# magcks/opencl_raytracer

Hardware: AMD Instinct MI355X
Metric: Mrays/s at 1920×1080 (bunny.off, sibenik.off); PGM bit-exact vs CPU (higher is better)
Workload: dtype f32; 1 GPU; bunny.off 1920x1080 -s 1 -a 3 (primary + 28 AO rays per hit sub-pixel), longest-axis BVH; rays_per_frame=34404360, primary_hits=1154670, parallelism=image bands x1, frames_in_flight=1, frame_launch=hipGraph replay, pgm_md5=e02eaeb53640206897ce798cda5cbd83, pgm_matches_golden=True, scene_bytes_on_device=20837632, scene_copies_on_device=1, triangles=70570, device=AMD Radeon Graphics

## Files before the change

include/rt_hip_debug.h:

```cpp
#ifndef RT_HIP_DEBUG_H
#define RT_HIP_DEBUG_H

#include "rt_hip_ring.h"

#ifdef __cplusplus
extern "C" {
#endif

double rt_total_kernel_ms(const rt_host *h);
float rt_last_ao_ms(const rt_host *h);
double rt_total_ao_ms(const rt_host *h);
uint64_t rt_kernel_launches(const rt_host *h);
void rt_reset_timers(rt_host *h);

int rt_ring_device_bytes(const rt_ring *r, uint64_t *scene_bytes, uint32_t *scene_copies, uint64_t *total_bytes);

int rt_ring_calibration(const rt_ring *r, float *ms_without, float *ms_with, int *prefetch_in_use);
int rt_set_ao_prefetch(rt_host *h, int on);

int rt_walk_entries(rt_host *h, uint32_t *tiles_hit, uint32_t *tiles_narrowed, double *mean_share, double *mean_packet_share);

int rt_ring_reset_clock(rt_ring *r);
int rt_ring_keep_frame_times(rt_ring *r, int on);
int rt_ring_frame_times(const rt_ring *r, uint64_t frame, float ms[4]);

int rt_ring_timers(rt_ring *r, double *kernel_ms, uint64_t *frames, double *ao_ms, uint64_t *ao_frames);
void rt_ring_reset_timers(rt_ring *r);

int rt_ring_cpu_times(const rt_ring *r, double *submit_s, double *wait_s, double *collect_s, uint64_t *frames);

int rt_ring_rccl_info(rt_ring *r, int *comm_ranks, int *rccl_version);
int rt_ring_rccl_self_test(rt_ring *r);

int rt_debug_measure_tile_costs(rt_host *h, uint32_t frames, int reorder);
int rt_debug_set_order_policy(rt_host *h, float heavy, float runway, float split_above);
int rt_debug_set_primary_split(rt_host *h, uint32_t above);
uint32_t rt_debug_tile_order_slots(rt_host *h);
uint32_t rt_debug_tiles(rt_host *h);
int rt_debug_tile_order(rt_host *h, uint32_t *order, uint32_t *constants24, uint32_t *tile_words, float *tile_costs);
int rt_debug_set_tile_order(rt_host *h, const uint32_t *order, uint32_t slots, const uint32_t *constants24);
int rt_debug_split_tiles(rt_host *h, uint32_t out[8]);
int rt_debug_set_cheap_claims(rt_host *h, float cheap_below);
int rt_debug_cheap_tiles(rt_host *h, uint32_t out[8]);

int rt_debug_prune_facts(rt_host *h, float *prune_margin, uint32_t *unpruned_bytes, uint32_t *primary_bytes);

int rt_debug_poison_hit_list(rt_host *h);

int rt_debug_set_views_chunk(rt_host *h, uint32_t max_views);
int rt_debug_last_views(rt_host *h, uint32_t *views, uint32_t *chunks, uint64_t *ao_points);

#define RT_DEBUG_NEAREST_NO_START 1u
#define RT_DEBUG_NEAREST_NO_PRUNE 2u
// ... 19 lines not shown
```

opencl_raytracer_amd/api.py:

```python
from __future__ import annotations

import ctypes as C
import weakref
import os
import sys
from typing import Optional

import numpy as np

_HERE = os.path.dirname(os.path.abspath(__file__))


def lib_path() -> str:
    return os.path.join(_HERE, os.environ.get("OCRT_LIB_DIR", "lib"), "libocrt_hip.so")


class RtError(RuntimeError):
    def __init__(self, code: int, message: str):
        super().__init__(f"[rt {code}] {message}")
        self.code = code
        self.message = message


RT_E_INVALID, RT_E_NO_DEVICE, RT_E_DEVICE, RT_E_STATE, RT_E_IO = -1, -2, -3, -4, -5
# ... 149 lines not shown
    "rt_ring_submit": (C.c_int, [C.c_void_p, C.POINTER(C.c_uint64)]),
    "rt_ring_collect": (C.c_int, [C.c_void_p, C.POINTER(C.c_uint64), C.POINTER(C.c_uint32), C.POINTER(C.c_void_p)]),
    "rt_ring_collect_into_device": (C.c_int, [C.c_void_p, C.c_void_p]),
    "rt_ring_step": (C.c_int, [C.c_void_p]),
    "rt_ring_run": (C.c_int, [C.c_void_p, C.c_uint32]),
    "rt_ring_drain": (C.c_int, [C.c_void_p]),
    "rt_ring_last_image_device": (C.c_int, [C.c_void_p, C.POINTER(C.c_void_p)]),
    "rt_ring_download_last": (C.c_int, [C.c_void_p, C.c_void_p]),
    "rt_ring_reset_clock": (C.c_int, [C.c_void_p]),
    "rt_ring_keep_frame_times": (C.c_int, [C.c_void_p, C.c_int]),
    "rt_ring_frame_times": (C.c_int, [C.c_void_p, C.c_uint64, C.POINTER(C.c_float)]),
    "rt_ring_timers": (C.c_int, [C.c_void_p, C.POINTER(C.c_double), C.POINTER(C.c_uint64), C.POINTER(C.c_double),
                                 C.POINTER(C.c_uint64)]),
    "rt_ring_reset_timers": (None, [C.c_void_p]),
    "rt_ring_cpu_times": (C.c_int, [C.c_void_p, C.POINTER(C.c_double), C.POINTER(C.c_double), C.POINTER(C.c_double),
                                    C.POINTER(C.c_uint64)]),
    "rt_rccl_available": (C.c_int, []),
    "rt_rccl_unique_id": (C.c_int, [C.c_void_p]),
    "rt_ring_attach_rccl": (C.c_int, [C.c_void_p, C.c_void_p]),
    "rt_ring_rccl_self_test": (C.c_int, [C.c_void_p]),
    "rt_print_info": (None, []),
    "rt_device_count": (C.c_int, []),
    "rt_debug_measure_tile_costs": (C.c_int, [C.c_void_p, C.c_uint32, C.c_int]),
    "rt_debug_set_order_policy": (C.c_int, [C.c_void_p, C.c_float, C.c_float, C.c_float]),
    "rt_debug_set_primary_split": (C.c_int, [C.c_void_p, C.c_uint32]),
    "rt_debug_tile_order_slots": (C.c_uint32, [C.c_void_p]),
    "rt_debug_tiles": (C.c_uint32, [C.c_void_p]),
    "rt_debug_tile_order": (C.c_int, [C.c_void_p, C.c_void_p, C.c_void_p, C.c_void_p, C.c_void_p]),
    "rt_debug_set_tile_order": (C.c_int, [C.c_void_p, C.c_void_p, C.c_uint32, C.c_void_p]),
    "rt_debug_split_tiles": (C.c_int, [C.c_void_p, C.c_void_p]),
    "rt_debug_set_cheap_claims": (C.c_int, [C.c_void_p, C.c_float]),
    "rt_debug_cheap_tiles": (C.c_int, [C.c_void_p, C.c_void_p]),
    "rt_debug_prune_facts": (C.c_int, [C.c_void_p, C.c_void_p, C.c_void_p, C.c_void_p]),
    "rt_debug_poison_hit_list": (C.c_int, [C.c_void_p]),
    "rt_debug_node_test_forms": (C.c_int, [C.c_int, C.c_void_p, C.c_uint32, C.c_void_p, C.c_uint32, C.c_void_p]),
    "rt_debug_set_views_chunk": (C.c_int, [C.c_void_p, C.c_uint32]),
    "rt_debug_last_views": (C.c_int, [C.c_void_p, C.POINTER(C.c_uint32), C.POINTER(C.c_uint32), C.POINTER(C.c_uint64)]),
    "rt_trace_closest": (C.c_int, [C.c_void_p, C.c_void_p, C.c_void_p, C.c_uint32, C.c_float, C.c_uint32, C.c_void_p]),
    "rt_trace_occluded": (C.c_int, [C.c_void_p, C.c_void_p, C.c_void_p, C.c_uint32, C.c_float, C.c_uint32, C.c_void_p]),
    "rt_trace_closest_device": (C.c_int, [C.c_void_p, C.c_void_p, C.c_void_p, C.c_uint32, C.c_float, C.c_uint32, C.c_void_p,
                                          C.c_void_p]),
    "rt_trace_occluded_device": (C.c_int, [C.c_void_p, C.c_void_p, C.c_void_p, C.c_uint32, C.c_float, C.c_uint32, C.c_void_p,
                                           C.c_void_p]),
    "rt_last_query_ms": (C.c_float, [C.c_void_p]),
    "rt_segments_occluded": (C.c_int, [C.c_void_p, C.c_void_p, C.c_void_p, C.c_uint32, C.c_float, C.c_float, C.c_uint32, C.c_void_p]),
    "rt_segments_closest": (C.c_int, [C.c_void_p, C.c_void_p, C.c_void_p, C.c_uint32, C.c_float, C.c_float, C.c_uint32, C.c_void_p]),
    "rt_segments_occluded_device": (C.c_int, [C.c_void_p, C.c_void_p, C.c_void_p, C.c_uint32, C.c_float, C.c_float, C.c_uint32,
                                              C.c_void_p, C.c_void_p]),
    "rt_segments_closest_device": (C.c_int, [C.c_void_p, C.c_void_p, C.c_void_p, C.c_uint32, C.c_float, C.c_float, C.c_uint32,
                                             C.c_void_p, C.c_void_p]),
    "rt_visibility_masks": (C.c_int, [C.c_void_p, C.c_void_p, C.c_uint32, C.c_void_p, C.c_uint32, C.c_float, C.c_float, C.c_uint32,
                                      C.c_void_p]),
    "rt_visibility_masks_device": (C.c_int, [C.c_void_p, C.c_void_p, C.c_uint32, C.c_void_p, C.c_uint32, C.c_float, C.c_float,
                                             C.c_uint32, C.c_void_p, C.c_void_p]),
    "rt_instances_segments_occluded": (C.c_int, [C.c_void_p, C.c_void_p, C.c_void_p, C.c_uint32, C.c_float, C.c_float, C.c_uint32,
                                                 C.c_void_p]),
    "rt_instances_segments_closest": (C.c_int, [C.c_void_p, C.c_void_p, C.c_void_p, C.c_uint32, C.c_float, C.c_float, C.c_uint32,
                                                C.c_void_p]),
    "rt_instances_segments_occluded_device": (C.c_int, [C.c_void_p, C.c_void_p, C.c_void_p, C.c_uint32, C.c_float, C.c_float, C.c_uint32,
                                                        C.c_void_p, C.c_void_p]),
    "rt_instances_segments_closest_device": (C.c_int, [C.c_void_p, C.c_void_p, C.c_void_p, C.c_uint32, C.c_float, C.c_float, C.c_uint32,
                                                       C.c_void_p, C.c_void_p]),
    "rt_instances_visibility_masks": (C.c_int, [C.c_void_p, C.c_void_p, C.c_uint32, C.c_void_p, C.c_uint32, C.c_float, C.c_float,
                                                C.c_uint32, C.c_void_p]),
    "rt_instances_visibility_masks_device": (C.c_int, [C.c_void_p, C.c_void_p, C.c_uint32, C.c_void_p, C.c_uint32, C.c_float, C.c_float,
                                                       C.c_uint32, C.c_void_p, C.c_void_p]),
# ... 591 lines not shown
        words, costs = np.zeros(tiles, np.uint32), np.zeros(tiles, np.float32)
        _check(lib.rt_debug_tile_order(self._h, order.ctypes.data, constants.ctypes.data, words.ctypes.data, costs.ctypes.data))
        return {"order": order, "constants": constants.reshape(8, 3), "words": words, "costs": costs}

    def set_tile_order(self, order, constants) -> None:
        order = np.ascontiguousarray(order, np.uint32)
        constants = np.ascontiguousarray(constants, np.uint32).reshape(24)
        _check(load_library().rt_debug_set_tile_order(self._h, order.ctypes.data, len(order), constants.ctypes.data))

    def split_tiles(self) -> np.ndarray:
        out = np.zeros(8, np.uint32)
        _check(load_library().rt_debug_split_tiles(self._h, out.ctypes.data))
        return out

    def set_cheap_claims(self, cheap_below: float) -> None:
        _check(load_library().rt_debug_set_cheap_claims(self._h, float(cheap_below)))

    def cheap_tiles(self) -> np.ndarray:
        out = np.zeros(8, np.uint32)
        _check(load_library().rt_debug_cheap_tiles(self._h, out.ctypes.data))
        return out

    def prune_facts(self) -> dict:
        margin, unpruned, primary = C.c_float(), C.c_uint32(), C.c_uint32()
        _check(load_library().rt_debug_prune_facts(self._h, C.byref(margin), C.byref(unpruned), C.byref(primary)))
        return {"prune_margin": float(margin.value), "unpruned_bytes": unpruned.value, "primary_bytes": primary.value}

    def walk_entries(self) -> dict:
        hit, narrowed, share, packet_share = C.c_uint32(), C.c_uint32(), C.c_double(), C.c_double()
        _check(load_library().rt_walk_entries(self._h, C.byref(hit), C.byref(narrowed), C.byref(share), C.byref(packet_share)))
        return {"tiles_hit": hit.value, "tiles_narrowed": narrowed.value, "mean_share": share.value,
                "mean_packet_share": packet_share.value}

    def stats(self) -> dict:
        s = _Stats()
        _check(load_library().rt_get_stats(self._h, C.byref(s)))
        return {k: int(getattr(s, k)) for k, _ in _Stats._fields_}

    @property
    def last_kernel_ms(self) -> float:
        return float(load_library().rt_last_kernel_ms(self._h))

    @property
    def total_kernel_ms(self) -> float:
        return float(load_library().rt_total_kernel_ms(self._h))

    @property
    def last_ao_ms(self) -> float:
        return float(load_library().rt_last_ao_ms(self._h))

    @property
    def total_ao_ms(self) -> float:
        return float(load_library().rt_total_ao_ms(self._h))

    @property
    def kernel_launches(self) -> int:
        return int(load_library().rt_kernel_launches(self._h))

    def reset_timers(self) -> None:
        load_library().rt_reset_timers(self._h)

    def trace_closest(self, origins, directions, max_distance: float = 100000.0, outputs=QUERY_OUTPUTS, sort: bool = True) -> dict:
        return self._trace(True, origins, directions, max_distance, tuple(outputs), sort)

    def trace_occluded(self, origins, directions, max_distance: float = 100000.0, sort: bool = True):
        return self._trace(False, origins, directions, max_distance, ("hit",), sort)["hit"]
# ... 668 lines not shown
```

opencl_raytracer_amd/csrc/c_api.cc:

```cpp
#include "../../include/rt_hip.h"
#include "../../include/rt_hip_ao.h"
#include "../../include/rt_hip_camera.h"
#include "../../include/rt_hip_directional.h"
#include "../../include/rt_hip_layers.h"
#include "../../include/rt_hip_debug.h"
#include "../../include/rt_hip_multihit.h"
#include "../../include/rt_hip_nearest.h"
#include "../../include/rt_hip_query.h"
#include "../../include/rt_hip_segment.h"
#include "../../include/rt_hip_instance_build.h"
#include "../../include/rt_hip_instance_directional.h"
#include "../../include/rt_hip_instance_multihit.h"
#include "../../include/rt_hip_instance_nearest.h"
#include "../../include/rt_hip_instance_segments.h"
#include "../../include/rt_hip_instance_views.h"
#include "../../include/rt_hip_instances.h"
#include "../../include/rt_hip_views.h"
#include "../../include/rt_hip_update.h"
#include "../../include/rt_hip_build.h"

#include <algorithm>
#include <hip/hip_runtime.h>

#include <cmath>
// ... 545 lines not shown

int rt_ring_set_calibration(rt_ring *r, int on) {
	if (!r)
		return fail(RT_E_INVALID, "null argument");
	r->ring->setCalibration(on != 0);
	return RT_OK;
}

int rt_ring_calibration(const rt_ring *r, float *ms_without, float *ms_with, int *prefetch_in_use) {
	if (!r)
		return fail(RT_E_INVALID, "null argument");
	if (ms_without)
		*ms_without = r->ring->calibrationMs()[0];
	if (ms_with)
		*ms_with = r->ring->calibrationMs()[1];
	if (prefetch_in_use)
		*prefetch_in_use = r->ring->aoPrefetch() ? 1 : 0;
	return RT_OK;
}

int rt_walk_entries(rt_host *h, uint32_t *tiles_hit, uint32_t *tiles_narrowed, double *mean_share, double *mean_packet_share) {
	if (!h)
		return fail(RT_E_INVALID, "null argument");
	return guarded([&] {
		const ocrt::DeviceRenderer::WalkEntries e = h->dev->walkEntries();
		if (tiles_hit)
			*tiles_hit = e.tiles_hit;
		if (tiles_narrowed)
			*tiles_narrowed = e.tiles_narrowed;
		if (mean_share)
			*mean_share = e.mean_share;
		if (mean_packet_share)
			*mean_packet_share = e.mean_packet_share;
	});
}

int rt_set_ao_prefetch(rt_host *h, int on) {
	if (!h)
		return fail(RT_E_INVALID, "null argument");
	return guarded([&] { h->dev->setAoPrefetch(on != 0); });
}

int rt_debug_measure_tile_costs(rt_host *h, uint32_t frames, int reorder) {
	if (!h)
		return fail(RT_E_INVALID, "null argument");
	return guarded([&] {
		h->dev->measureTileCosts(frames, reorder != 0);
	});
}

int rt_debug_set_primary_split(rt_host *h, uint32_t above) {
	if (!h)
		return fail(RT_E_INVALID, "null argument");
	return guarded([&] { h->dev->setPrimarySplit(above); });
}

int rt_debug_set_order_policy(rt_host *h, float heavy, float runway, float split_above) {
	if (!h)
		return fail(RT_E_INVALID, "null argument");
	return guarded([&] { h->dev->setOrderPolicy(heavy, runway, split_above); });
}

uint32_t rt_debug_tile_order_slots(rt_host *h) {
	if (!h)
		return 0;
	std::vector<uint32_t> order, constants, words;
// ... 1285 lines not shown
```

opencl_raytracer_amd/csrc/device_renderer.cc:

```cpp
#include "device_internal.h"

#include <algorithm>
#include <array>
#include <atomic>
#include <chrono>

#include <hip/hip_runtime.h>

#include <cstddef>
#include <cstdio>
#include <cstdlib>
#include <cstring>
#include <mutex>
#include <sstream>

namespace ocrt {


int visible_device_count() {
	int count = 0;
	if (hipGetDeviceCount(&count) != hipSuccess)
		return 0;
	return count;
}
// ... 430 lines not shown
	OCRT_HIP(hipStreamSynchronize((hipStream_t) stream));
	const double whole = (double) kp.node_count * sizeof(NodeRec);
	double sum = 0.0, sum_packets = 0.0;
	unsigned long long packets = 0;
	const size_t tiles_per_piece = std::max<size_t>(1, ((size_t) 32 << 20) / (stride * 2 * sizeof(uint32_t)));
	std::vector<uint32_t> ranges;
	for (size_t first = 0; first < tile_count; first += tiles_per_piece) {
		const size_t count = std::min(tiles_per_piece, tile_count - first);
		ranges.resize(count * stride * 2);
		OCRT_HIP(hipMemcpyAsync(ranges.data(), (const uint32_t *) d_tile_entry + first * stride * 2, ranges.size() * sizeof(uint32_t), hipMemcpyDeviceToHost,
		                        (hipStream_t) stream));
		OCRT_HIP(hipStreamSynchronize((hipStream_t) stream));
		for (size_t t = first; t < first + count; ++t) {
			if ((words[t] & 0xFFu) == 0u)
				continue;
			++out.tiles_hit;
			const uint32_t *const of_tile = &ranges[2 * stride * (t - first)];
			const double bytes = std::min(whole, (double) of_tile[1]) - (double) of_tile[0];
			out.tiles_narrowed += of_tile[0] != 0u || bytes < whole;
			sum += bytes / whole;
			const bool per_direction = (words[t] & 0xFFu) == 64u && kp.ao_mode == AO_UNIFORM && stride > 1;
			for (size_t k = 1; k <= kp.ao_dirs; ++k) {
				const uint32_t *const r = per_direction ? of_tile + 2 * k : of_tile;
				sum_packets += (std::min(whole, (double) r[1]) - (double) r[0]) / whole;
				++packets;
			}
		}
	}
	out.mean_share = out.tiles_hit ? sum / out.tiles_hit : 1.0;
	out.mean_packet_share = packets ? sum_packets / (double) packets : 1.0;
	return out;
}

void DeviceRenderer::expectFrames(uint64_t frames) {
	const bool before = expected_frames >= FRAMES_WORTH_INTERVALS, after = frames >= FRAMES_WORTH_INTERVALS;
	if (before != after && scene_ready)
		requireFramePath("expectFrames");
	expected_frames = frames;
	if (before == after || !scene_ready)
		return;
	std::shared_ptr<const DeviceScene> scene = scene_on_device;
	std::shared_ptr<DeviceScene> mine = scene_of_my_own;
	adopt(std::move(scene));
	scene_of_my_own = std::move(mine);
}

void DeviceRenderer::setAoPrefetch(bool on) {
	if (on == ao_prefetch)
		return;
	ao_prefetch = on;
	++scene_version;
}

bool DeviceRenderer::calibrateAoPrefetch(float *ms_without, float *ms_with) {
	if (!scene_ready)
		throw std::logic_error("calibration before upload");
	requireFramePath("calibration");
	const bool has_ao = kp.ao_mode == AO_UNIFORM && kp.ao_dirs > 0 && tile_count > 0 && kp.fast_walk && kp.walk_scale > 0.0f;
	float median[2] = { 0.0f, 0.0f };
	if (has_ao) {
		const bool before = ao_prefetch;
		std::vector<float> samples[2];
		for (int round = 0; round < 6; ++round)
			for (int form = 0; form < 2; ++form) {
				ao_prefetch = form != 0;
				enqueueRender();
// ... 321 lines not shown
```

opencl_raytracer_amd/csrc/device_renderer.h:

```cpp
#pragma once
#include <array>
#include <cstdint>
#include <memory>
#include <stdexcept>
#include <string>
#include <vector>

#include "device_types.h"
#include "ray_tracer.h"
#include "scene_pack.h"

namespace ocrt {

struct DeviceError : std::runtime_error {
	using std::runtime_error::runtime_error;
};

int visible_device_count();
void warm_up_device(int device);

class DeviceScene {
	public:
		static std::shared_ptr<DeviceScene> create(int device, const PackedScene &scene, const RayTracer::Options &options, bool for_a_stream = true,
		                                           const float *eye = nullptr);
// ... 75 lines not shown
		void setRefitGroup(uint32_t nodes) { refit_group = nodes; }
		uint32_t refitGroup() const { return refit_group; }
		void setCamera(const CameraPose &pose);
		bool cameraIsSet() const { return pose_set; }
		const CameraPose &camera() const { return pose; }

		void enqueueRender();
		void enqueueResize();
		void enqueueResizeInto(void *device_u8);
		void enqueueFrame(void *device_u8 = nullptr);
		void prepareFrame(void *device_u8 = nullptr);
		void setGraphMode(bool on) { graph_mode = on; }
		bool sceneReady() const { return scene_ready; }
		bool graphMode() const { return graph_mode; }
		void synchronize();
		void waitForStream();
		void setEpochEvent(void *event) { epoch_event = event; }
		void setKeepStamps(bool on) { keep_stamps = on; }
		const float *lastFrameTimes() const { return last_times; }

		const void *deviceBands() const { return d_u8; }
		void *streamHandle() const { return stream; }
		void setDeviceShare(unsigned hosts) {
			device_share = hosts < 1u ? 1u : hosts;
			kp.shared_device = device_share > 1u ? 1 : 0;
		}
		void setAoPrefetch(bool on);
		struct WalkEntries {
			uint32_t tiles_hit, tiles_narrowed;
			double mean_share;
			double mean_packet_share;
		};
		WalkEntries walkEntries() const;
		bool aoPrefetch() const { return ao_prefetch; }
		static constexpr uint64_t FRAMES_WORTH_INTERVALS = 16;
		static constexpr float CHEAP_BELOW_DEFAULT = 0.15f;
		void expectFrames(uint64_t frames);
		uint64_t expectedFrames() const { return expected_frames; }
		bool walkIntervalsInUse() const { return intervals_in_use; }
		bool measureTileCosts(unsigned frames = 2, bool reorder = true);
		void takeOrderFrom(const DeviceRenderer &other);
		bool orderIsMeasured() const { return tile_cost.size() == tile_count && tile_count != 0; }
		void setOrderPolicy(float heavy, float runway, float split_above = -1.0f);
		void setPrimarySplit(uint32_t above);
		void poisonHitList();
		void tileOrder(std::vector<uint32_t> &order, std::vector<uint32_t> &constants, std::vector<uint32_t> &words, std::vector<float> &cost) const;
		void setTileOrder(const std::vector<uint32_t> &order, const std::vector<uint32_t> &constants);
		const std::array<uint32_t, XCD_GROUPS> &splitTiles() const { return split_tiles; }
		const std::array<uint32_t, XCD_GROUPS> &cheapTiles() const { return cheap_tiles; }
		void setCheapClaims(float cheap_below);
		bool calibrateAoPrefetch(float *ms_without = nullptr, float *ms_with = nullptr);
		uint32_t aoWorkgroups() const {
			if (scene_beyond_caches)
				return compute_units * 8u;
			return device_share >= 6u ? compute_units * 3u : device_share > 1u ? compute_units * 9u / 2u : compute_units * 8u;
		}
		uint32_t globalRowOf(uint32_t local_row) const;

		void downloadFloat(float *host_image);
		void downloadResizedLocal(unsigned char *host);
		void downloadResizedFull(unsigned char *host);

		void setStream(void *hip_stream);
		void usePrivateStream();

		RenderStats stats();
// ... 136 lines not shown
```

opencl_raytracer_amd/csrc/kernels/entry.hip.h:

```cpp
#pragma once
#include "common.hip.h"

namespace ocrt {

constexpr uint32_t ENTRY_WAVES = 4;
__global__ __launch_bounds__(64 * ENTRY_WAVES) void entry_kernel(const NodeRec *__restrict__ walk, const HitRec *__restrict__ hits,
                                                                 const uint32_t *__restrict__ tile_hits, const uint32_t *__restrict__ tile_base,
                                                                 const float4 *__restrict__ ao_table, uint2 *__restrict__ tile_entry,
                                                                 uint32_t tiles, uint32_t stride, int32_t uniform_table,
                                                                 float max_distance) {
	__shared__ float origin[ENTRY_WAVES][3][64];
	__shared__ float frame[ENTRY_WAVES][9][64];
	const uint32_t wave = threadIdx.x >> 6, lane = threadIdx.x & 63u;
	const uint32_t tile = blockIdx.x * ENTRY_WAVES + wave;
	if (tile >= tiles)
		return;
	const uint32_t hit_count = tile_hits[tile] & 0xFFu;
	uint2 *const out = tile_entry + (size_t) tile * stride;
	const uint32_t whole = walk[0].skip / (uint32_t) sizeof(NodeRec);
	if (lane < hit_count) {
		const HitRec rec = hits[(size_t) tile_base[tile] + lane];
		const float nx = rec.nx, ny = rec.ny, nz = rec.nz;
		const float eps = 1.0f / 100000.0f;
		origin[wave][0][lane] = rec.ox + nx * eps;
// ... 38 lines not shown
			return !(box.lo[0] - box.hi[0] > hi[0] || box.lo[0] + box.hi[0] < lo[0] || box.lo[1] - box.hi[1] > hi[1] || box.lo[1] + box.hi[1] < lo[1] ||
			         box.lo[2] - box.hi[2] > hi[2] || box.lo[2] + box.hi[2] < lo[2]);
		};
		uint32_t begin = 0u, end = whole ? whole : 1u;
		if (!odd && (j == 0u || one_direction)) {
			uint32_t n = 0u;
			while (skip_of(n) > 1u) {
				uint32_t first = 0u, index = 0u, others = 0u;
				for (uint32_t c = n + 1u; c < n + skip_of(n); c += skip_of(c)) {
					if (first)
						others += meets(c) ? 1u : 0u;
					else {
						++index;
						if (meets(c))
							first = c;
					}
				}
				if (first == 0u) {
					n += skip_of(n);
					break;
				}
				if (index == 1u && others != 0u)
					break;
				n = first;
			}
			begin = n;
			n = 0u;
			while (skip_of(n) > 1u) {
				uint32_t last = 0u;
				for (uint32_t c = n + 1u; c < n + skip_of(n); c += skip_of(c))
					if (meets(c))
						last = c;
				if (last == 0u) {
					end = n;
					break;
				}
				end = last + skip_of(last);
				n = last;
			}
			if (begin > end)
				begin = end;
		}
		out[j] = make_uint2(begin * (uint32_t) sizeof(NodeRec), end * (uint32_t) sizeof(NodeRec));
	}
}

}
```

opencl_raytracer_amd/csrc/kernels/walk.hip.h:

```cpp
#pragma once
#include "common.hip.h"

namespace ocrt {

__device__ __forceinline__ bool exact_box(const float4 lo, const float4 hi, const Ray &ray, float max_distance, bool alive,
                                          uint32_t at, uint32_t skip, uint32_t &mine) {
	const bool here = alive && mine == at;
	const bool box = here && slab_hit(lo, hi, ray, max_distance);
	mine = here ? (box ? at + 1u : at + skip) : mine;
	return box;
}

struct SignMasks {
	unsigned long long x, y, z;
};
__device__ __forceinline__ SignMasks sign_masks(const Ray &r) {
	SignMasks m;
	m.x = wave_ballot(r.ix >= 0.0f);
	m.y = wave_ballot(r.iy >= 0.0f);
	m.z = wave_ballot(r.iz >= 0.0f);
	return m;
}

typedef unsigned int u32x8 __attribute__((ext_vector_type(8)));
// ... 33 lines not shown
	"\tv_max_f32 v58, 1, v58\n"                    \
	"\tv_min_f32 v61, %[below], v61\n"             \
	"\tv_max3_f32 v56, v56, v57, v58\n"            \
	"\tv_min3_f32 v59, v59, v60, v61\n"            \
	"\tv_cmp_le_f32 vcc, v56, v59\n"
#define OCRT_TEST_MIXED(LX, LY, LZ, HX, HY, HZ)    \
	"\tv_fma_f32 v56, " LX ", %[ix], %[oix]\n"     \
	"\tv_fma_f32 v57, " HX ", %[ix], %[oix]\n"     \
	"\tv_fma_f32 v58, " LY ", %[iy], %[oiy]\n"     \
	"\tv_fma_f32 v59, " HY ", %[iy], %[oiy]\n"     \
	"\tv_fma_f32 v60, " LZ ", %[iz], %[oiz]\n"     \
	"\tv_fma_f32 v61, " HZ ", %[iz], %[oiz]\n"     \
	"\tv_cndmask_b32 v62, v57, v56, %[px]\n"       \
	"\tv_cndmask_b32 v56, v56, v57, %[px]\n"       \
	"\tv_cndmask_b32 v57, v59, v58, %[py]\n"       \
	"\tv_cndmask_b32 v58, v58, v59, %[py]\n"       \
	"\tv_cndmask_b32 v59, v61, v60, %[pz]\n"       \
	"\tv_cndmask_b32 v60, v60, v61, %[pz]\n"       \
	"\tv_max_f32 v59, 1, v59\n"                    \
	"\tv_min_f32 v60, %[below], v60\n"             \
	"\tv_max3_f32 v62, v62, v57, v59\n"            \
	"\tv_min3_f32 v56, v56, v58, v60\n"            \
	"\tv_cmp_le_f32 vcc, v62, v56\n"
#define OCRT_TEST_CE_SCALED(CX, CY, CZ, E_XY, E_ZW)                                                                   \
	"\tv_fma_f32 v56, " CX ", %[ix], %[oix]\n"                                                                        \
	"\tv_fma_f32 v58, " CY ", %[iy], %[oiy]\n"                                                                        \
	"\tv_fma_f32 v60, " CZ ", %[iz], %[oiz]\n"                                                                        \
	"\tv_pk_fma_f32 v[56:57], " E_XY ", %[axy], v[56:57] op_sel:[0,0,0] op_sel_hi:[0,0,0] neg_lo:[1,0,0]\n"           \
	"\tv_pk_fma_f32 v[58:59], " E_XY ", %[axy], v[58:59] op_sel:[1,1,0] op_sel_hi:[1,1,0] neg_lo:[1,0,0]\n"           \
	"\tv_pk_fma_f32 v[60:61], " E_ZW ", %[azw], v[60:61] op_sel:[0,0,0] op_sel_hi:[0,0,0] neg_lo:[1,0,0] clamp\n"     \
	"\tv_max3_f32 v56, v56, v58, v60\n"                                                                               \
	"\tv_min3_f32 v57, v57, v59, v61\n"                                                                               \
	"\tv_cmp_lt_f32 vcc, v56, v57\n"
#define OCRT_WALK_LEAF(LEAF, NOW, NEXT)                 \
	"\ts_cmp_eq_u32 " LEAF ", -2\n"                     \
	"\ts_cbranch_scc1 .Lw_over_%=\n"                    \
	"\ts_bcnt1_i32_b64 s46, s[44:45]\n"                 \
	"\ts_add_u32 %[stops], %[stops], 1\n"               \
	"\ts_cmp_ge_u32 s46, %[batch_below]\n"              \
	"\ts_cbranch_scc1 " NOW "\n"                        \
	"\tv_mbcnt_lo_u32_b32 v56, s44, 0\n"                \
	"\tv_mbcnt_hi_u32_b32 v56, s45, v56\n"              \
	"\tv_add_u32 v56, %[waiting], v56\n"                \
	"\tv_lshl_add_u32 v56, v56, 2, %[list]\n"           \
	"\tv_or_b32 v57, " LEAF ", %[tag]\n"                \
	"\ts_mov_b64 s[42:43], exec\n"                      \
	"\ts_mov_b64 exec, s[44:45]\n"                      \
	"\tds_write_b32 v56, v57\n"                         \
	"\ts_mov_b64 exec, s[42:43]\n"                      \
	"\ts_add_u32 %[waiting], %[waiting], s46\n"         \
	"\ts_cmp_ge_u32 %[waiting], 64\n"                   \
	"\ts_cbranch_scc1 .Lw_full_%=\n"                    \
	"\ts_branch " NEXT "\n"
#define OCRT_PF_NONE ""
#define OCRT_PF_SUCCESSORS                                    \
	"\ts_cmp_lg_u32 s63, -1\n"                               \
	"\ts_cbranch_scc1 .Lw_no_pf_%=\n"                        \
	"\ts_add_u32 s46, %[at], 32\n"                           \
	"\ts_load_dword s47, %[base], s46\n"                     \
	"\ts_add_u32 s46, %[at], s59\n"                          \
	"\ts_load_dword s47, %[base], s46\n"                     \
	".Lw_no_pf_%=:\n"
#define OCRT_HEAD_NONE ""
#define OCRT_HEAD_END "\ts_cmp_ge_u32 %[at], %[end]\n\ts_cbranch_scc1 .Lw_over_wait_%=\n"
#define OCRT_WALK_ASM(HEAD, TEST_A, TEST_B, PF_B)           \
	"\ts_branch .Lw_node_%=\n"                              \
	".Lw_miss_a_%=:\n"                                      \
	"\ts_add_u32 %[at], %[at], s51\n"                       \
	".Lw_node_%=:\n"                                        \
	"\ts_load_dwordx16 s[48:63], %[base], %[at]\n"          \
	HEAD                                                    \
	"\ts_waitcnt lgkmcnt(0)\n"                              \
	TEST_A                                                  \
	"\ts_and_b64 s[44:45], vcc, %[alive]\n"                 \
	"\ts_cbranch_scc0 .Lw_miss_a_%=\n"                      \
	"\ts_cmp_lg_u32 s55, -1\n"                              \
	"\ts_cbranch_scc1 .Lw_leaf_a_%=\n"                      \
	".Lw_next_b_%=:\n"                                      \
	"\ts_add_u32 %[at], %[at], 32\n"                        \
	PF_B                                                    \
	TEST_B                                                  \
	"\ts_and_b64 s[44:45], vcc, %[alive]\n"                 \
	"\ts_cbranch_scc0 .Lw_miss_b_%=\n"                      \
	"\ts_cmp_lg_u32 s63, -1\n"                              \
	"\ts_cbranch_scc1 .Lw_leaf_b_%=\n"                      \
	".Lw_next_a_%=:\n"                                      \
	"\ts_add_u32 %[at], %[at], 32\n"                        \
	"\ts_branch .Lw_node_%=\n"                              \
	".Lw_miss_b_%=:\n"                                      \
	"\ts_add_u32 %[at], %[at], s59\n"                       \
	"\ts_branch .Lw_node_%=\n"                              \
	".Lw_leaf_a_%=:\n"                                      \
	OCRT_WALK_LEAF("s55", ".Lw_now_a_%=", ".Lw_next_b_%=")  \
	".Lw_now_a_%=:\n"                                       \
	"\ts_mov_b32 %[leaf], s55\n"                            \
	"\ts_branch .Lw_now_%=\n"                               \
	".Lw_leaf_b_%=:\n"                                      \
	OCRT_WALK_LEAF("s63", ".Lw_now_b_%=", ".Lw_next_a_%=")  \
	".Lw_now_b_%=:\n"                                       \
	"\ts_mov_b32 %[leaf], s63\n"                            \
	".Lw_now_%=:\n"                                         \
	"\ts_mov_b64 %[hit], s[44:45]\n"                        \
	"\ts_mov_b32 %[status], 1\n"                            \
	"\ts_branch .Lw_out_%=\n"                               \
	".Lw_full_%=:\n"                                        \
	"\ts_mov_b32 %[status], 2\n"                            \
	"\ts_branch .Lw_out_%=\n"                               \
	".Lw_over_wait_%=:\n"                                   \
	"\ts_waitcnt lgkmcnt(0)\n"                              \
	".Lw_over_%=:\n"                                        \
	"\ts_mov_b32 %[status], 0\n"                            \
	".Lw_out_%=:\n"
#define OCRT_WALK_CLOBBERS                                                                                              \
	"s42", "s43", "s44", "s45", "s46", "s47", "s48", "s49", "s50", "s51", "s52", "s53", "s54", "s55", "s56", "s57", "s58", \
	    "s59", "s60", "s61", "s62", "s63", "v56", "v57", "v58", "v59", "v60", "v61", "v62", "vcc", "scc", "memory"
#define OCRT_NEAR_P(LO, HI) LO
#define OCRT_NEAR_N(LO, HI) HI
#define OCRT_FAR_P(LO, HI) HI
#define OCRT_FAR_N(LO, HI) LO
#define OCRT_WALK_COHERENT(TEST, X, Y, Z, PF)                                                                               \
	asm volatile(OCRT_WALK_ASM(OCRT_HEAD_NONE, TEST(OCRT_NEAR_##X("s48", "s52"), OCRT_NEAR_##Y("s49", "s53"),              \
	                                OCRT_NEAR_##Z("s50", "s54"), OCRT_FAR_##X("s48", "s52"),                               \
	                                OCRT_FAR_##Y("s49", "s53"), OCRT_FAR_##Z("s50", "s54")),                               \
	                           TEST(OCRT_NEAR_##X("s56", "s60"), OCRT_NEAR_##Y("s57", "s61"),                              \
	                                OCRT_NEAR_##Z("s58", "s62"), OCRT_FAR_##X("s56", "s60"),                               \
	                                OCRT_FAR_##Y("s57", "s61"), OCRT_FAR_##Z("s58", "s62")), PF)                           \
	             : [at] "+s"(at), [waiting] "+s"(waiting), [stops] "+s"(leaf_stops), [hit] "=&s"(hit_mask),               \
	               [leaf] "=&s"(leaf), [status] "=&s"(status)                                                            \
	             : [base] "s"(walk_ptr), [alive] "s"(alive_mask), [below] "v"(below), [batch_below] "s"(batch_below),     \
	               [list] "s"(list_lds_address), [tag] "v"(lane_tag), [ix] "v"(ray.ix), [iy] "v"(ray.iy), [iz] "v"(ray.iz), \
	               [oix] "v"(ray.oix), [oiy] "v"(ray.oiy), [oiz] "v"(ray.oiz)                                             \
	             : OCRT_WALK_CLOBBERS)

#define OCRT_WALK_MIXED(TEST, PF)                                                                                         \
	asm volatile(OCRT_WALK_ASM(OCRT_HEAD_NONE, TEST("s48", "s49", "s50", "s52", "s53", "s54"), TEST("s56", "s57", "s58", "s60", "s61", "s62"), PF) \
	             : [at] "+s"(at), [waiting] "+s"(waiting), [stops] "+s"(leaf_stops), [hit] "=&s"(hit_mask),               \
	               [leaf] "=&s"(leaf), [status] "=&s"(status)                                                            \
	             : [base] "s"(walk_ptr), [alive] "s"(alive_mask), [below] "v"(below), [batch_below] "s"(batch_below),     \
	               [px] "s"(sign.x), [py] "s"(sign.y), [pz] "s"(sign.z), [list] "s"(list_lds_address), [tag] "v"(lane_tag), \
	               [ix] "v"(ray.ix), [iy] "v"(ray.iy), [iz] "v"(ray.iz), [oix] "v"(ray.oix), [oiy] "v"(ray.oiy),          \
	               [oiz] "v"(ray.oiz)                                                                                    \
	             : OCRT_WALK_CLOBBERS)
#define OCRT_WALK_MIXED_CE(TEST, PF)                                                                                      \
	asm volatile(OCRT_WALK_ASM(OCRT_HEAD_END, TEST("s48", "s49", "s50", "s[52:53]", "s[54:55]"), TEST("s56", "s57", "s58", "s[60:61]", "s[62:63]"), PF) \
	             : [at] "+s"(at), [waiting] "+s"(waiting), [stops] "+s"(leaf_stops), [hit] "=&s"(hit_mask),               \
	               [leaf] "=&s"(leaf), [status] "=&s"(status)                                                            \
	             : [base] "s"(walk_ptr), [alive] "s"(alive_mask), [end] "s"(walk_end), [batch_below] "s"(batch_below),    \
	               [list] "s"(list_lds_address), [tag] "v"(lane_tag),                                                      \
	               [ix] "v"(ray.ix), [iy] "v"(ray.iy), [iz] "v"(ray.iz), [oix] "v"(ray.oix), [oiy] "v"(ray.oiy),          \
	               [oiz] "v"(ray.oiz), [axy] "v"(abs_xy), [azw] "v"(abs_zw)                                               \
	             : OCRT_WALK_CLOBBERS)
#define OCRT_WALK_SWITCH(COHERENT_TEST, MIXED_TEST, PF)                 \
	switch (variant) {                                                  \
	case 0u: OCRT_WALK_COHERENT(COHERENT_TEST, N, N, N, PF); break;     \
	case 1u: OCRT_WALK_COHERENT(COHERENT_TEST, P, N, N, PF); break;     \
	case 2u: OCRT_WALK_COHERENT(COHERENT_TEST, N, P, N, PF); break;     \
	case 3u: OCRT_WALK_COHERENT(COHERENT_TEST, P, P, N, PF); break;     \
	case 4u: OCRT_WALK_COHERENT(COHERENT_TEST, N, N, P, PF); break;     \
	case 5u: OCRT_WALK_COHERENT(COHERENT_TEST, P, N, P, PF); break;     \
	case 6u: OCRT_WALK_COHERENT(COHERENT_TEST, N, P, P, PF); break;     \
	case 7u: OCRT_WALK_COHERENT(COHERENT_TEST, P, P, P, PF); break;     \
	default: MIXED_TEST; break;                                         \
	}

constexpr uint32_t WALK_MIXED = 8u;
typedef float f32x2 __attribute__((ext_vector_type(2)));
template <bool SCALED, bool PREFETCH = false>
__device__ __forceinline__ uint32_t walk_collect(uint32_t variant, const float4 *walk_ptr, uint32_t &at, const WalkRay &ray,
                                                 const SignMasks &sign, float below, unsigned long long alive_mask,
                                                 unsigned long long &hit_mask, uint32_t &leaf, uint32_t &waiting,
                                                 uint32_t &leaf_stops, uint32_t list_lds_address, uint32_t lane_tag,
                                                 uint32_t batch_below, uint32_t walk_end = 0xFFFFFFFFu) {
	(void) walk_end;
	uint32_t status;
	if (SCALED) {
		(void) sign;
		(void) variant;
		const f32x2 abs_xy = { __builtin_fabsf(ray.ix), __builtin_fabsf(ray.iy) };
		const f32x2 abs_zw = { __builtin_fabsf(ray.iz), __builtin_fabsf(ray.iz) };
		if (PREFETCH) {
			OCRT_WALK_MIXED_CE(OCRT_TEST_CE_SCALED, OCRT_PF_SUCCESSORS);
		} else {
			OCRT_WALK_MIXED_CE(OCRT_TEST_CE_SCALED, OCRT_PF_NONE);
		}
	} else {
		OCRT_WALK_SWITCH(OCRT_TEST_COHERENT, OCRT_WALK_MIXED(OCRT_TEST_MIXED, OCRT_PF_NONE), OCRT_PF_NONE)
	}
	return status;
}

__device__ __forceinline__ uint32_t walk_variant(const SignMasks &sign, unsigned long long alive_mask) {
	const unsigned long long x = sign.x & alive_mask, y = sign.y & alive_mask, z = sign.z & alive_mask;
	bool coherent = (x == 0ull || x == alive_mask) && (y == 0ull || y == alive_mask) && (z == 0ull || z == alive_mask);
#ifdef OCRT_ALWAYS_MIXED
	coherent = false;
#endif
	return coherent ? (x != 0ull ? 1u : 0u) | (y != 0ull ? 2u : 0u) | (z != 0ull ? 4u : 0u) : WALK_MIXED;
}

__device__ __forceinline__ bool exact_leaf_gate(const float4 lo, const float4 hi, const Ray &r, float below) {
	const float x0 = (lo.x - r.ox) * r.ix, x1 = (hi.x - r.ox) * r.ix;
	const float y0 = (lo.y - r.oy) * r.iy, y1 = (hi.y - r.oy) * r.iy;
	const float z0 = (lo.z - r.oz) * r.iz, z1 = (hi.z - r.oz) * r.iz;
	const bool px = r.ix >= 0.0f, py = r.iy >= 0.0f, pz = r.iz >= 0.0f;
	const float tiny = __uint_as_float(1u);
	const float t_near = fmaxf(fmaxf(px ? x0 : x1, py ? y0 : y1), fmaxf(pz ? z0 : z1, tiny));
// ... 53 lines not shown
			const int owner = (int) (pair >> 26);
			const Ray ray = with_origin();
			Ray theirs;
			theirs.ox = __shfl(ray.ox, owner); theirs.oy = __shfl(ray.oy, owner); theirs.oz = __shfl(ray.oz, owner);
			theirs.dx = __shfl(ray.dx, owner); theirs.dy = __shfl(ray.dy, owner); theirs.dz = __shfl(ray.dz, owner);
			theirs.ix = theirs.iy = theirs.iz = 0.0f;
			const uint32_t pair_leaf = pair & 0x03FFFFFFu;
			const float4 *rec = (const float4 *) ((const char *) tris_ptr + pair_leaf * LEAF_BYTES);
			bool accepted = false;
			if (lane < n)
				accepted = tri_any_hit(rec[2], rec[3], rec[4], rec[5], rec[1].w, theirs);
			const bool any_accepted = wave_ballot(accepted) != 0ull;
#ifdef OCRT_STAMPS
			prof[5] += n;
			count_event(0u, (uint32_t) __popcll(wave_ballot(accepted)));
			count_event(n == 64u ? 1u : 2u, 1u);
			count_event(3u, n == 64u ? 0u : n);
			count_event(5u, any_accepted ? 0u : 1u);
#endif
			if (any_accepted) {
				theirs.ix = __shfl(ray.ix, owner); theirs.iy = __shfl(ray.iy, owner); theirs.iz = __shfl(ray.iz, owner);
				bool gate = false;
				if (accepted) {
					const float4 lo = rec[0], hi = rec[1];
					gate = exact_leaf_gate(lo, hi, theirs, below);
					if (gate)
						atomicOr(&batch.occluded_bits[owner >> 5], 1u << (owner & 31));
				}
#ifdef OCRT_STAMPS
				prof[6] += (unsigned long long) __popcll(wave_ballot(gate));
#endif
				wave_lds_sync();
				const uint32_t bits = batch.occluded_bits[lane >> 5];
				if (alive && ((bits >> (lane & 31u)) & 1u)) {
					atomicAdd(occluded, 1u);
					alive = false;
				}
				wave_lds_sync();
				if (lane < 2u)
					batch.occluded_bits[lane] = 0u;
				alive_mask = wave_ballot(alive);
			}
#ifdef OCRT_STAMPS
			prof[1] += __builtin_amdgcn_s_memrealtime() - tb0;
			prof[3] += 1;
#endif
		};
		const uint32_t list_lds_address = (uint32_t) __builtin_amdgcn_readfirstlane((int) (uint32_t) (uintptr_t) &batch.entry[0]);
		const SignMasks sign{ 0ull, 0ull, 0ull };
		const uint32_t variant = WALK_MIXED;
		uint32_t at = copy + entry_begin;
		const uint32_t whole = count * 32u;
		const uint32_t end = copy + (entry_end < whole ? entry_end : whole);
		const WalkRay walk_ray = tame ? make_walk_ray(with_origin(), walk_scale, true) : make_walk_ray(with_origin(), walk_scale);
		const uint32_t lane_tag = fresh_lane() << 26;
		while (alive_mask != 0ull && at < end) {
			uint32_t leaf = 0u;
			unsigned long long hit_mask = 0ull;
#ifdef OCRT_STAMPS
			const unsigned long long tw0 = __builtin_amdgcn_s_memrealtime();
#endif
			const uint32_t status = walk_collect<true, PREFETCH>(variant, walk_ptr, at, walk_ray, sign, below, alive_mask, hit_mask, leaf,
			                                           waiting, leaf_stops, list_lds_address, lane_tag, batch_below, end);
#ifdef OCRT_STAMPS
			prof[0] += __builtin_amdgcn_s_memrealtime() - tw0;
			prof[2] += 1;
#endif
			if (status == 0u)
				break;
			if (status == 1u) {
				const float4 *rec = tris_ptr + LEAF_F4 * leaf;
				const float4 q0 = rec[2], q1 = rec[3], q2 = rec[4], q3 = rec[5];
				const float inv_d = rec[1].w;
				const Ray ray = with_origin();
				bool accepted = false;
				if ((hit_mask >> fresh_lane()) & 1ull)
					accepted = tri_any_hit(q0, q1, q2, q3, inv_d, ray);
				const bool any_accepted = wave_ballot(accepted) != 0ull;
#ifdef OCRT_STAMPS
				count_event(4u, 1u);
				count_event(6u, any_accepted ? 0u : 1u);
#endif
				if (any_accepted) {
					const float4 lo = rec[0], hi = rec[1];
					if (accepted && exact_leaf_gate(lo, hi, ray, below)) {
						atomicAdd(occluded, 1u);
						alive = false;
					}
					alive_mask = wave_ballot(alive);
				}
			} else {
				run_batch(64u);
				waiting -= 64u;
				const uint32_t me = fresh_lane();
				if (me < waiting)
					batch.entry[me] = batch.entry[64u + me];
			}
			at += 32u;
		}
		if (waiting != 0u)
			run_batch(waiting);
#ifdef OCRT_STAMPS
		prof[4] += leaf_stops;
#endif
		return;
	}
	const Ray ray = ray_in;
	exact_walk(nodes_ptr, count, ray, max_distance, alive, [&](uint32_t leaf, bool box) {
		const float4 *tri = tris_ptr + LEAF_F4 * leaf + LEAF_TRI_F4;
		const float4 q0 = tri[0], q1 = tri[1], q2 = tri[2], q3 = tri[3];
		if (box) {
			const TriResult tr = tri_eval<false>(q0, q1, q2, q3, ray);
			if (tr.accepted) {
				atomicAdd(occluded, 1u);
				alive = false;
			}
		}
		return wave_ballot(alive) == 0ull;
	});
}

}
```

Measured before the change: 36550 Mrays/s.

## Streamline any-hit walk loop and trim interval ends after inner nodes

```diff
diff --git a/include/rt_hip_debug.h b/include/rt_hip_debug.h
--- a/include/rt_hip_debug.h
+++ b/include/rt_hip_debug.h
@@ -19,6 +19,7 @@
 int rt_set_ao_prefetch(rt_host *h, int on);
 
 int rt_walk_entries(rt_host *h, uint32_t *tiles_hit, uint32_t *tiles_narrowed, double *mean_share, double *mean_packet_share);
+int rt_debug_walk_interval_ends(rt_host *h, uint32_t out[6]);
 
 int rt_ring_reset_clock(rt_ring *r);
 int rt_ring_keep_frame_times(rt_ring *r, int on);
diff --git a/opencl_raytracer_amd/api.py b/opencl_raytracer_amd/api.py
--- a/opencl_raytracer_amd/api.py
+++ b/opencl_raytracer_amd/api.py
@@ -205,6 +205,7 @@
     "rt_debug_set_cheap_claims": (C.c_int, [C.c_void_p, C.c_float]),
     "rt_debug_cheap_tiles": (C.c_int, [C.c_void_p, C.c_void_p]),
     "rt_debug_prune_facts": (C.c_int, [C.c_void_p, C.c_void_p, C.c_void_p, C.c_void_p]),
+    "rt_debug_walk_interval_ends": (C.c_int, [C.c_void_p, C.c_void_p]),
     "rt_debug_poison_hit_list": (C.c_int, [C.c_void_p]),
     "rt_debug_node_test_forms": (C.c_int, [C.c_int, C.c_void_p, C.c_uint32, C.c_void_p, C.c_uint32, C.c_void_p]),
     "rt_debug_set_views_chunk": (C.c_int, [C.c_void_p, C.c_uint32]),
@@ -862,6 +863,12 @@
         return {"tiles_hit": hit.value, "tiles_narrowed": narrowed.value, "mean_share": share.value,
                 "mean_packet_share": packet_share.value}
 
+    def walk_interval_ends(self) -> dict:
+        out = np.zeros(6, np.uint32)
+        _check(load_library().rt_debug_walk_interval_ends(self._h, out.ctypes.data))
+        keys = ("intervals", "whole_array", "after_leaf", "after_inner", "last_is_leaf", "last_is_inner")
+        return {k: int(v) for k, v in zip(keys, out)}
+
     def stats(self) -> dict:
         s = _Stats()
         _check(load_library().rt_get_stats(self._h, C.byref(s)))
diff --git a/opencl_raytracer_amd/csrc/c_api.cc b/opencl_raytracer_amd/csrc/c_api.cc
--- a/opencl_raytracer_amd/csrc/c_api.cc
+++ b/opencl_raytracer_amd/csrc/c_api.cc
@@ -601,6 +601,20 @@
 			*mean_share = e.mean_share;
 		if (mean_packet_share)
 			*mean_packet_share = e.mean_packet_share;
+	});
+}
+
+int rt_debug_walk_interval_ends(rt_host *h, uint32_t out[6]) {
+	if (!h || !out)
+		return fail(RT_E_INVALID, "null argument");
+	return guarded([&] {
+		const ocrt::DeviceRenderer::IntervalEnds e = h->dev->walkIntervalEnds();
+		out[0] = e.intervals;
+		out[1] = e.whole_array;
+		out[2] = e.after_leaf;
+		out[3] = e.after_inner;
+		out[4] = e.last_is_leaf;
+		out[5] = e.last_is_inner;
 	});
 }
 
diff --git a/opencl_raytracer_amd/csrc/device_renderer.cc b/opencl_raytracer_amd/csrc/device_renderer.cc
--- a/opencl_raytracer_amd/csrc/device_renderer.cc
+++ b/opencl_raytracer_amd/csrc/device_renderer.cc
@@ -486,6 +486,61 @@
 	return out;
 }
 
+DeviceRenderer::IntervalEnds DeviceRenderer::walkIntervalEnds() const {
+	if (!scene_ready)
+		throw std::logic_error("walkIntervalEnds: no scene on the device");
+	useDevice();
+	IntervalEnds out{ 0, 0, 0, 0, 0, 0 };
+	const bool has_ao = kp.ao_mode != AO_NONE && kp.ao_dirs > 0;
+	const void *const walk = scene_on_device->buffers().walk;
+	if (tile_count == 0 || !has_ao || kp.node_count == 0 || !walk || kp.walk_ce_bytes == 0)
+		return out;
+	const size_t stride = kp.entry_stride;
+	const uint32_t nodes = kp.node_count;
+	std::vector<NodeRec> records(nodes);
+	std::vector<uint32_t> words(tile_count), ranges(tile_count * stride * 2);
+	OCRT_HIP(hipStreamSynchronize((hipStream_t) stream));
+	OCRT_HIP(hipMemcpyAsync(records.data(), (const char *) walk + kp.walk_ce_bytes, records.size() * sizeof(NodeRec), hipMemcpyDeviceToHost, (hipStream_t) stream));
+	OCRT_HIP(hipMemcpyAsync(words.data(), d_tile_hits, words.size() * sizeof(uint32_t), hipMemcpyDeviceToHost, (hipStream_t) stream));
+	OCRT_HIP(hipMemcpyAsync(ranges.data(), d_tile_entry, ranges.size() * sizeof(uint32_t), hipMemcpyDeviceToHost, (hipStream_t) stream));
+	OCRT_HIP(hipStreamSynchronize((hipStream_t) stream));
+	const auto skip_of = [&](uint32_t n) { return records[n].skip / (uint32_t) sizeof(NodeRec); };
+	const uint32_t none = 0xFFFFFFFFu;
+	std::vector<uint32_t> innermost(nodes + 1, none);
+	for (uint32_t n = 0; n < nodes; ++n)
+		if (skip_of(n) > 1u && n + skip_of(n) <= nodes)
+			innermost[n + skip_of(n)] = n;
+	for (size_t t = 0; t < tile_count; ++t) {
+		const uint32_t hits = words[t] & 0xFFu;
+		if (hits == 0u)
+			continue;
+		const bool per_direction = hits == 64u && kp.ao_mode == AO_UNIFORM && stride > 1;
+		for (size_t k = 1; k <= (per_direction ? (size_t) kp.ao_dirs : 1); ++k) {
+			const uint32_t *const r = &ranges[2 * (stride * t + (per_direction ? k : 0))];
+			++out.intervals;
+			if (r[1] / sizeof(NodeRec) >= nodes) {
+				++out.whole_array;
+				continue;
+			}
+			const uint32_t begin = r[0] / (uint32_t) sizeof(NodeRec), end = r[1] / (uint32_t) sizeof(NodeRec);
+			if (begin >= end) {
+				--out.intervals;
+				continue;
+			}
+			if (skip_of(end - 1u) > 1u) {
+				++out.after_inner;
+				continue;
+			}
+			++out.after_leaf;
+			if (innermost[end] != none && innermost[end] >= begin)
+				++out.last_is_inner;
+			else
+				++out.last_is_leaf;
+		}
+	}
+	return out;
+}
+
 void DeviceRenderer::expectFrames(uint64_t frames) {
 	const bool before = expected_frames >= FRAMES_WORTH_INTERVALS, after = frames >= FRAMES_WORTH_INTERVALS;
 	if (before != after && scene_ready)
diff --git a/opencl_raytracer_amd/csrc/device_renderer.h b/opencl_raytracer_amd/csrc/device_renderer.h
--- a/opencl_raytracer_amd/csrc/device_renderer.h
+++ b/opencl_raytracer_amd/csrc/device_renderer.h
@@ -131,6 +131,15 @@
 			double mean_packet_share;
 		};
 		WalkEntries walkEntries() const;
+		struct IntervalEnds {
+			uint32_t intervals;
+			uint32_t whole_array;
+			uint32_t after_leaf;
+			uint32_t after_inner;
+			uint32_t last_is_leaf;
+			uint32_t last_is_inner;
+		};
+		IntervalEnds walkIntervalEnds() const;
 		bool aoPrefetch() const { return ao_prefetch; }
 		static constexpr uint64_t FRAMES_WORTH_INTERVALS = 16;
 		static constexpr float CHEAP_BELOW_DEFAULT = 0.15f;
diff --git a/opencl_raytracer_amd/csrc/kernels/entry.hip.h b/opencl_raytracer_amd/csrc/kernels/entry.hip.h
--- a/opencl_raytracer_amd/csrc/kernels/entry.hip.h
+++ b/opencl_raytracer_amd/csrc/kernels/entry.hip.h
@@ -94,7 +94,8 @@
 					if (meets(c))
 						last = c;
 				if (last == 0u) {
-					end = n;
+					if (n == 0u || skip_of(n - 1u) == 1u)
+						end = n;
 					break;
 				}
 				end = last + skip_of(last);
diff --git a/opencl_raytracer_amd/csrc/kernels/walk.hip.h b/opencl_raytracer_amd/csrc/kernels/walk.hip.h
--- a/opencl_raytracer_amd/csrc/kernels/walk.hip.h
+++ b/opencl_raytracer_amd/csrc/kernels/walk.hip.h
@@ -89,11 +89,15 @@
 	"\tv_max3_f32 v56, v56, v58, v60\n"                                                                               \
 	"\tv_min3_f32 v57, v57, v59, v61\n"                                                                               \
 	"\tv_cmp_lt_f32 vcc, v56, v57\n"
-#define OCRT_WALK_LEAF(LEAF, NOW, NEXT)                 \
+#define OCRT_COUNT_STOPS "\ts_add_u32 %[stops], %[stops], 1\n"
+#define OCRT_COUNT_NONE ""
+#define OCRT_NARROW_MOV "\ts_mov_b64 s[42:43], exec\n\ts_mov_b64 exec, s[44:45]\n"
+#define OCRT_NARROW_AND "\ts_and_saveexec_b64 s[42:43], s[44:45]\n"
+#define OCRT_WALK_LEAF(LEAF, NOW, NEXT, COUNT, NARROW)  \
 	"\ts_cmp_eq_u32 " LEAF ", -2\n"                     \
 	"\ts_cbranch_scc1 .Lw_over_%=\n"                    \
 	"\ts_bcnt1_i32_b64 s46, s[44:45]\n"                 \
-	"\ts_add_u32 %[stops], %[stops], 1\n"               \
+	COUNT                                               \
 	"\ts_cmp_ge_u32 s46, %[batch_below]\n"              \
 	"\ts_cbranch_scc1 " NOW "\n"                        \
 	"\tv_mbcnt_lo_u32_b32 v56, s44, 0\n"                \
@@ -101,8 +105,7 @@
 	"\tv_add_u32 v56, %[waiting], v56\n"                \
 	"\tv_lshl_add_u32 v56, v56, 2, %[list]\n"           \
 	"\tv_or_b32 v57, " LEAF ", %[tag]\n"                \
-	"\ts_mov_b64 s[42:43], exec\n"                      \
-	"\ts_mov_b64 exec, s[44:45]\n"                      \
+	NARROW                                              \
 	"\tds_write_b32 v56, v57\n"                         \
 	"\ts_mov_b64 exec, s[42:43]\n"                      \
 	"\ts_add_u32 %[waiting], %[waiting], s46\n"         \
@@ -120,13 +123,22 @@
 	".Lw_no_pf_%=:\n"
 #define OCRT_HEAD_NONE ""
 #define OCRT_HEAD_END "\ts_cmp_ge_u32 %[at], %[end]\n\ts_cbranch_scc1 .Lw_over_wait_%=\n"
-#define OCRT_WALK_ASM(HEAD, TEST_A, TEST_B, PF_B)           \
+#define OCRT_ENTRY_NONE ""
+#define OCRT_ENTRY_ALIVE "\ts_cmp_eq_u64 %[alive], 0\n\ts_cbranch_scc1 .Lw_over_%=\n"
+#define OCRT_DESCEND_CHECKED ""
+#define OCRT_DESCEND_UNCHECKED                                \
+	"\ts_add_u32 %[at], %[at], 32\n"                          \
+	"\ts_load_dwordx16 s[48:63], %[base], %[at]\n"            \
+	"\ts_branch .Lw_wait_%=\n"
+#define OCRT_WALK_ASM(ENTRY, HEAD, DESCEND, COUNT, NARROW, TEST_A, TEST_B, PF_B) \
+	ENTRY                                                   \
 	"\ts_branch .Lw_node_%=\n"                              \
 	".Lw_miss_a_%=:\n"                                      \
 	"\ts_add_u32 %[at], %[at], s51\n"                       \
 	".Lw_node_%=:\n"                                        \
 	"\ts_load_dwordx16 s[48:63], %[base], %[at]\n"          \
 	HEAD                                                    \
+	".Lw_wait_%=:\n"                                        \
 	"\ts_waitcnt lgkmcnt(0)\n"                              \
 	TEST_A                                                  \
 	"\ts_and_b64 s[44:45], vcc, %[alive]\n"                 \
@@ -141,6 +153,7 @@
 	"\ts_cbranch_scc0 .Lw_miss_b_%=\n"                      \
 	"\ts_cmp_lg_u32 s63, -1\n"                              \
 	"\ts_cbranch_scc1 .Lw_leaf_b_%=\n"                      \
+	DESCEND                                                 \
 	".Lw_next_a_%=:\n"                                      \
 	"\ts_add_u32 %[at], %[at], 32\n"                        \
 	"\ts_branch .Lw_node_%=\n"                              \
@@ -148,12 +161,12 @@
 	"\ts_add_u32 %[at], %[at], s59\n"                       \
 	"\ts_branch .Lw_node_%=\n"                              \
 	".Lw_leaf_a_%=:\n"                                      \
-	OCRT_WALK_LEAF("s55", ".Lw_now_a_%=", ".Lw_next_b_%=")  \
+	OCRT_WALK_LEAF("s55", ".Lw_now_a_%=", ".Lw_next_b_%=", COUNT, NARROW)  \
 	".Lw_now_a_%=:\n"                                       \
 	"\ts_mov_b32 %[leaf], s55\n"                            \
 	"\ts_branch .Lw_now_%=\n"                               \
 	".Lw_leaf_b_%=:\n"                                      \
-	OCRT_WALK_LEAF("s63", ".Lw_now_b_%=", ".Lw_next_a_%=")  \
+	OCRT_WALK_LEAF("s63", ".Lw_now_b_%=", ".Lw_next_a_%=", COUNT, NARROW)  \
 	".Lw_now_b_%=:\n"                                       \
 	"\ts_mov_b32 %[leaf], s63\n"                            \
 	".Lw_now_%=:\n"                                         \
@@ -168,6 +181,17 @@
 	".Lw_over_%=:\n"                                        \
 	"\ts_mov_b32 %[status], 0\n"                            \
 	".Lw_out_%=:\n"
+#define OCRT_WALK_PLAIN(TEST_A, TEST_B, PF) \
+	OCRT_WALK_ASM(OCRT_ENTRY_NONE, OCRT_HEAD_NONE, OCRT_DESCEND_CHECKED, OCRT_COUNT_STOPS, OCRT_NARROW_MOV, TEST_A, TEST_B, PF)
+#ifdef OCRT_STAMPS
+#define OCRT_ANY_HIT_COUNT OCRT_COUNT_STOPS
+#define OCRT_ANY_HIT_STOPS , [stops] "+s"(leaf_stops)
+#else
+#define OCRT_ANY_HIT_COUNT OCRT_COUNT_NONE
+#define OCRT_ANY_HIT_STOPS
+#endif
+#define OCRT_WALK_ANY_HIT(TEST_A, TEST_B, PF) \
+	OCRT_WALK_ASM(OCRT_ENTRY_ALIVE, OCRT_HEAD_END, OCRT_DESCEND_UNCHECKED, OCRT_ANY_HIT_COUNT, OCRT_NARROW_AND, TEST_A, TEST_B, PF)
 #define OCRT_WALK_CLOBBERS                                                                                              \
 	"s42", "s43", "s44", "s45", "s46", "s47", "s48", "s49", "s50", "s51", "s52", "s53", "s54", "s55", "s56", "s57", "s58", \
 	    "s59", "s60", "s61", "s62", "s63", "v56", "v57", "v58", "v59", "v60", "v61", "v62", "vcc", "scc", "memory"
@@ -176,7 +200,7 @@
 #define OCRT_FAR_P(LO, HI) HI
 #define OCRT_FAR_N(LO, HI) LO
 #define OCRT_WALK_COHERENT(TEST, X, Y, Z, PF)                                                                               \
-	asm volatile(OCRT_WALK_ASM(OCRT_HEAD_NONE, TEST(OCRT_NEAR_##X("s48", "s52"), OCRT_NEAR_##Y("s49", "s53"),              \
+	asm volatile(OCRT_WALK_PLAIN(TEST(OCRT_NEAR_##X("s48", "s52"), OCRT_NEAR_##Y("s49", "s53"),              \
 	                                OCRT_NEAR_##Z("s50", "s54"), OCRT_FAR_##X("s48", "s52"),                               \
 	                                OCRT_FAR_##Y("s49", "s53"), OCRT_FAR_##Z("s50", "s54")),                               \
 	                           TEST(OCRT_NEAR_##X("s56", "s60"), OCRT_NEAR_##Y("s57", "s61"),                              \
@@ -190,7 +214,7 @@
 	             : OCRT_WALK_CLOBBERS)
 
 #define OCRT_WALK_MIXED(TEST, PF)                                                                                         \
-	asm volatile(OCRT_WALK_ASM(OCRT_HEAD_NONE, TEST("s48", "s49", "s50", "s52", "s53", "s54"), TEST("s56", "s57", "s58", "s60", "s61", "s62"), PF) \
+	asm volatile(OCRT_WALK_PLAIN(TEST("s48", "s49", "s50", "s52", "s53", "s54"), TEST("s56", "s57", "s58", "s60", "s61", "s62"), PF) \
 	             : [at] "+s"(at), [waiting] "+s"(waiting), [stops] "+s"(leaf_stops), [hit] "=&s"(hit_mask),               \
 	               [leaf] "=&s"(leaf), [status] "=&s"(status)                                                            \
 	             : [base] "s"(walk_ptr), [alive] "s"(alive_mask), [below] "v"(below), [batch_below] "s"(batch_below),     \
@@ -199,10 +223,10 @@
 	               [oiz] "v"(ray.oiz)                                                                                    \
 	             : OCRT_WALK_CLOBBERS)
 #define OCRT_WALK_MIXED_CE(TEST, PF)                                                                                      \
-	asm volatile(OCRT_WALK_ASM(OCRT_HEAD_END, TEST("s48", "s49", "s50", "s[52:53]", "s[54:55]"), TEST("s56", "s57", "s58", "s[60:61]", "s[62:63]"), PF) \
-	             : [at] "+s"(at), [waiting] "+s"(waiting), [stops] "+s"(leaf_stops), [hit] "=&s"(hit_mask),               \
-	               [leaf] "=&s"(leaf), [status] "=&s"(status)                                                            \
-	             : [base] "s"(walk_ptr), [alive] "s"(alive_mask), [end] "s"(walk_end), [batch_below] "s"(batch_below),    \
+	asm volatile(OCRT_WALK_ANY_HIT(TEST("s48", "s49", "s50", "s[52:53]", "s[54:55]"), TEST("s56", "s57", "s58", "s[60:61]", "s[62:63]"), PF) \
+	             : [at] "+s"(at), [waiting] "+s"(waiting), [batch_below] "+s"(batch_below), [hit] "=&s"(hit_mask),        \
+	               [leaf] "=&s"(leaf), [status] "=&s"(status) OCRT_ANY_HIT_STOPS                                         \
+	             : [base] "s"(walk_ptr), [alive] "s"(alive_mask), [end] "s"(walk_end),                                    \
 	               [list] "s"(list_lds_address), [tag] "v"(lane_tag),                                                      \
 	               [ix] "v"(ray.ix), [iy] "v"(ray.iy), [iz] "v"(ray.iz), [oix] "v"(ray.oix), [oiy] "v"(ray.oiy),          \
 	               [oiz] "v"(ray.oiz), [axy] "v"(abs_xy), [azw] "v"(abs_zw)                                               \
@@ -227,8 +251,9 @@
                                                  const SignMasks &sign, float below, unsigned long long alive_mask,
                                                  unsigned long long &hit_mask, uint32_t &leaf, uint32_t &waiting,
                                                  uint32_t &leaf_stops, uint32_t list_lds_address, uint32_t lane_tag,
-                                                 uint32_t batch_below, uint32_t walk_end = 0xFFFFFFFFu) {
+                                                 uint32_t &batch_below, uint32_t walk_end = 0xFFFFFFFFu) {
 	(void) walk_end;
+	(void) leaf_stops;
 	uint32_t status;
 	if (SCALED) {
 		(void) sign;
@@ -348,14 +373,13 @@
 #endif
 				wave_lds_sync();
 				const uint32_t bits = batch.occluded_bits[lane >> 5];
-				if (alive && ((bits >> (lane & 31u)) & 1u)) {
+				const bool gone = ((alive_mask >> lane) & 1ull) && ((bits >> (lane & 31u)) & 1u);
+				if (gone)
 					atomicAdd(occluded, 1u);
-					alive = false;
-				}
 				wave_lds_sync();
 				if (lane < 2u)
 					batch.occluded_bits[lane] = 0u;
-				alive_mask = wave_ballot(alive);
+				alive_mask &= ~wave_ballot(gone);
 			}
 #ifdef OCRT_STAMPS
 			prof[1] += __builtin_amdgcn_s_memrealtime() - tb0;
@@ -370,20 +394,19 @@
 		const uint32_t end = copy + (entry_end < whole ? entry_end : whole);
 		const WalkRay walk_ray = tame ? make_walk_ray(with_origin(), walk_scale, true) : make_walk_ray(with_origin(), walk_scale);
 		const uint32_t lane_tag = fresh_lane() << 26;
-		while (alive_mask != 0ull && at < end) {
+		uint32_t status;
+		do {
 			uint32_t leaf = 0u;
 			unsigned long long hit_mask = 0ull;
 #ifdef OCRT_STAMPS
 			const unsigned long long tw0 = __builtin_amdgcn_s_memrealtime();
 #endif
-			const uint32_t status = walk_collect<true, PREFETCH>(variant, walk_ptr, at, walk_ray, sign, below, alive_mask, hit_mask, leaf,
-			                                           waiting, leaf_stops, list_lds_address, lane_tag, batch_below, end);
+			status = walk_collect<true, PREFETCH>(variant, walk_ptr, at, walk_ray, sign, below, alive_mask, hit_mask, leaf,
+			                                      waiting, leaf_stops, list_lds_address, lane_tag, batch_below, end);
 #ifdef OCRT_STAMPS
 			prof[0] += __builtin_amdgcn_s_memrealtime() - tw0;
 			prof[2] += 1;
 #endif
-			if (status == 0u)
-				break;
 			if (status == 1u) {
 				const float4 *rec = tris_ptr + LEAF_F4 * leaf;
 				const float4 q0 = rec[2], q1 = rec[3], q2 = rec[4], q3 = rec[5];
@@ -399,13 +422,12 @@
 #endif
 				if (any_accepted) {
 					const float4 lo = rec[0], hi = rec[1];
-					if (accepted && exact_leaf_gate(lo, hi, ray, below)) {
+					const bool gone = accepted && exact_leaf_gate(lo, hi, ray, below);
+					if (gone)
 						atomicAdd(occluded, 1u);
-						alive = false;
-					}
-					alive_mask = wave_ballot(alive);
+					alive_mask &= ~wave_ballot(gone);
 				}
-			} else {
+			} else if (status == 2u) {
 				run_batch(64u);
 				waiting -= 64u;
 				const uint32_t me = fresh_lane();
@@ -413,7 +435,7 @@
 					batch.entry[me] = batch.entry[64u + me];
 			}
 			at += 32u;
-		}
+		} while (status != 0u);
 		if (waiting != 0u)
 			run_batch(waiting);
 #ifdef OCRT_STAMPS
```

Result: faster. 37950 Mrays/s (median of 6 runs) (+3.8%).
